# sandeep06011991/OCC-GNN

Measured on AMD Instinct MI355X. Metric: sampled_edges_per_sec, higher is better.
Workload: dtype u32; 1 GPU; products-like synthetic (N=2449029, mean degree 50.5, pareto degrees, seed 0), GraphSAGE fanout 15/10/5 (layer 0 = seeds' hop), minibatch 1024, 4 parts (v % 4), engine-only (sample+slice); streams=128, round_overlap=True, device_lists=int32 (host exports widen to the reference's int64), engine_device_bytes=16549793524

## Files before the change

occ-gnn_amd/csrc/cslicer_hip.hip:

```cpp
#include <hip/hip_runtime.h>

#include <cstdarg>
#include <cstdio>
#include <cstdlib>
#include <cstring>
#include <algorithm>
#include <deque>
#include <vector>

#include "cslicer_hip.h"

namespace {

constexpr uint32_t UNSET = 0xFFFFFFFFu;

constexpr int TN = 256;
#ifdef CSL_OCC7
#define CSL_LB256 __launch_bounds__(256)
#else
#define CSL_LB256 __launch_bounds__(256, 8)
#endif
constexpr int CSL_MAX_SETS = 4;
constexpr int NW = TN / 64;
#ifndef CSL_TPB
// ... 37 lines not shown
       KN_EMIT, KN_SELFIN, KN_MT, KN_EDGES, KN_DUPSEEDS, KN_SELFIN_DEGREE };
const char* const kKernelNames[CSL_NUM_KERNELS] = {"k_seeds",   "k_degree", "k_scan_need", "k_sample",
                                                   "k_scan_buckets", "k_scatter", "k_bucket", "k_count",
                                                   "k_scan_lists", "k_emit",  "k_selfin",  "k_mt19937_fill",
                                                   "k_graph", "k_dupseeds", "k_selfin_degree"};

struct LArgs {
  const unsigned long long* rowinfo;
  const uint32_t* off32;
  const uint32_t* indices;
  const uint8_t* wl;
  uint32_t N, P;
  const uint32_t* ring;
  unsigned long long ring_mask, gen_lo, gen_hi;
  unsigned long long* rngpos;
  unsigned long long* rngbase;
  unsigned long long* acc;
  const uint32_t* fr_in;
  uint32_t* fr_out;
  size_t fr_in_stride, fr_out_stride;
  uint32_t fr_out_cap;
  unsigned long long* ninfo;
  uint32_t* hasedge;
  uint32_t* selfpos;
  uint32_t* firstpos;
  size_t fcap;
  uint32_t* cand;
  uint8_t* cflag;
  uint32_t* crank;
  uint2* queue;
  size_t ccap;
  uint32_t* nbk;
  uint32_t* bcnt;
  uint32_t* bcur;
  uint32_t nbmax;
  uint32_t* tcnt;
  uint32_t tmax, nk;
  uint32_t* fsize;
  csl_sample_meta* meta;
  int* arena;
  size_t arena_stride;
  size_t list_base[CSL_NUM_LISTS];
  uint32_t layer, fanout, W;
  unsigned long long wmagic;
  uint32_t S;
  uint32_t tpb;
  uint32_t* boff;
  uint32_t* ticket;
  uint32_t pmagic;
  uint32_t pmask;
  uint32_t last;
  uint32_t* dupflag;
  uint32_t* seedrep;
  uint32_t* dupfirst;
  uint32_t* dupout;
  size_t fcap0;
  unsigned long long* rngend;
  uint32_t* candk;
  uint32_t graph;
  uint8_t* ecnt;
  uint32_t* srcpos;
  uint32_t* tcur;
};

constexpr uint32_t SELF_BIT = 0x80000000u;
constexpr int kNoReplaceMaxFanout = 64;

__device__ __forceinline__ uint32_t mod_parts(const LArgs& a, uint32_t v) {
  uint32_t r = v - __umulhi(v, a.pmagic) * a.P;
  if (r >= a.P) r -= a.P;
  if (r >= a.P) r -= a.P;
  return r;
}
__device__ __forceinline__ uint32_t owner(const LArgs& a, uint32_t v) {
  return a.wl ? (uint32_t)a.wl[v] : mod_parts(a, v);
}
__device__ __forceinline__ unsigned long long row_lookup(const LArgs& a, uint32_t v) {
  if (a.off32) {
    const uint32_t lo = a.off32[v], hi = a.off32[v + 1];
    return ((unsigned long long)lo << 24) | (unsigned long long)(hi - lo);
  }
  return a.rowinfo[v];
}
__device__ __forceinline__ uint32_t lane_id() { return threadIdx.x & 63; }
__device__ __forceinline__ uint32_t div_w(const LArgs& a, uint32_t c) {
  return (uint32_t)(((unsigned long long)c * a.wmagic) >> 40);
}
__device__ __forceinline__ bool xcd_block_at(const LArgs& a, uint32_t id, uint32_t grid, uint32_t& x, uint32_t& s) {
  const uint32_t groups = (a.S + 7u) >> 3;
  const uint32_t per_stream = grid / (8u * groups);
  const uint32_t j = id >> 3;
  const uint32_t sl = j / per_stream;
  x = j - sl * per_stream;
  s = sl * 8u + (id & 7u);
  return s < a.S;
}
__device__ __forceinline__ bool xcd_block(const LArgs& a, uint32_t& x, uint32_t& s) {
  return xcd_block_at(a, blockIdx.x, gridDim.x, x, s);
}
__device__ __forceinline__ void st_sc1(uint32_t* p, uint32_t v) {
  __hip_atomic_store(p, v, __ATOMIC_RELAXED, __HIP_MEMORY_SCOPE_AGENT);
}
__device__ __forceinline__ uint32_t ld_sc1(const uint32_t* p) {
  return __hip_atomic_load(p, __ATOMIC_RELAXED, __HIP_MEMORY_SCOPE_AGENT);
}
__device__ __forceinline__ bool last_block_of_stream(uint32_t* ticket, uint32_t expected) {
  __shared__ uint32_t s_last;
  asm volatile("s_waitcnt vmcnt(0)" ::: "memory");
  __syncthreads();
  if (threadIdx.x == 0) {
    const uint32_t t = __hip_atomic_fetch_add(ticket, 1u, __ATOMIC_RELAXED, __HIP_MEMORY_SCOPE_AGENT);
    s_last = t == expected - 1u;
    if (t == expected - 1u) {
      st_sc1(ticket, 0u);
      __builtin_amdgcn_fence(__ATOMIC_ACQUIRE, "agent");
      asm volatile("s_waitcnt vmcnt(0)" ::: "memory");
    }
  }
  __syncthreads();
  return s_last != 0u;
}
__device__ __forceinline__ unsigned long long lt_mask() {
  return (1ull << lane_id()) - 1ull;
}
__device__ __forceinline__ uint32_t bucket_of(uint32_t v, uint32_t nb) {
  return __umulhi(v * 0x9E3779B1u, nb);
}
__device__ __forceinline__ uint32_t pass_of(uint32_t v, uint32_t npass) {
  uint32_t x = v * 0x27D4EB2Fu;
  x ^= x >> 13;
  return __umulhi(x * 0x165667B1u, npass);
}
__device__ __forceinline__ uint32_t slot_of(uint32_t v) {
  uint32_t x = v * 0x85EBCA6Bu;
  x ^= x >> 15;
  x *= 0xC2B2AE35u;
  return x >> (32 - HLOG);
}

__device__ __forceinline__ uint32_t wave_excl_scan(uint32_t x, uint32_t& total) {
  uint32_t incl = x;
  for (int o = 1; o < 64; o <<= 1) {
    uint32_t y = __shfl_up(incl, o);
    if ((int)lane_id() >= o) incl += y;
  }
  total = __shfl(incl, 63);
  return incl - x;
}

__device__ __forceinline__ uint32_t wave_incl_scan_dpp(uint32_t x) {
  int v = (int)x;
  v += __builtin_amdgcn_update_dpp(0, v, 0x111, 0xf, 0xf, false);
  v += __builtin_amdgcn_update_dpp(0, v, 0x112, 0xf, 0xf, false);
  v += __builtin_amdgcn_update_dpp(0, v, 0x114, 0xf, 0xf, false);
  v += __builtin_amdgcn_update_dpp(0, v, 0x118, 0xf, 0xf, false);
  v += __builtin_amdgcn_update_dpp(0, v, 0x142, 0xa, 0xf, false);
  v += __builtin_amdgcn_update_dpp(0, v, 0x143, 0xc, 0xf, false);
  return (uint32_t)v;
}
__device__ __forceinline__ uint32_t spread4(uint32_t x) { return ((x & 0xFu) * 0x00204081u) & 0x01010101u; }

constexpr int SCAN_CH = 12;

template <int PHASE>
__device__ __forceinline__ void scan_body(const LArgs& a, const int s) {
  const uint32_t F = ld_sc1(&a.fsize[s * (CSL_MAX_LAYERS + 1) + a.layer]);
// ... 336 lines not shown
      run += h;
      if (bx == 0) boff[b] = grun;
      grun += gcnt[b];
    }
    if (bx == 0 && n == TN - 1) boff[nb] = grun;
  }
  __syncthreads();
  for (uint32_t k0 = n; k0 < cnt; k0 += TN * CU) {
    uint32_t v[CU];
#pragma unroll
    for (int u = 0; u < CU; u++) v[u] = k0 + u * TN < cnt ? cand[k0 + u * TN] : UNSET;
#pragma unroll
    for (int u = 0; u < CU; u++) {
      if (v[u] == UNSET) continue;
      const uint32_t c = (uint32_t)base + k0 + u * TN;
      const uint32_t i = div_w(a, c);
      const uint32_t b = bucket_of(v[u], nb);
      const uint32_t p = s_loff[b] + atomicAdd(&s_hist[b], 1u);
      s_stage[p] = make_uint2(v[u], c == i * W ? (SELF_BIT | i) : c);
    }
  }
  __syncthreads();
  uint2* q = a.queue + (size_t)s * a.ccap;
  const uint32_t staged = s_loff[nb - 1] + s_hist[nb - 1];
  for (uint32_t k = n; k < staged; k += TN) {
    const uint2 e = s_stage[k];
    const uint32_t b = bucket_of(e.x, nb);
    q[s_gbase[b] + (k - s_loff[b])] = e;
  }
}

__device__ __forceinline__ uint32_t ht_find(const uint32_t* h_key, uint32_t val) {
  uint32_t h = slot_of(val);
  for (uint32_t probes = 0; probes < (uint32_t)HCAP; probes++) {
    const uint32_t k = h_key[h];
    if (k == val) return h;
    if (k == UNSET) return UNSET;
    h = (h + 1) & (HCAP - 1);
  }
  return UNSET;
}

#ifndef CSL_BT
#define CSL_BT 512
#endif
#ifndef CSL_RC
#define CSL_RC 4
#endif
constexpr int BT = CSL_BT;
constexpr int RC = CSL_RC;

__device__ __forceinline__ uint32_t ht_insert(uint32_t* h_key, uint32_t val) {
  uint32_t h = slot_of(val);
  for (uint32_t probes = 0; probes < (uint32_t)HCAP; probes++) {
    uint32_t kk = h_key[h];
    if (kk == UNSET) kk = atomicCAS(&h_key[h], UNSET, val);
    if (kk == UNSET || kk == val) return h;
    h = (h + 1) & (HCAP - 1);
  }
  return UNSET;
}

#ifndef CSL_BPB
#define CSL_BPB 4
#endif
constexpr int BPB = CSL_BPB;

__device__ unsigned long long g_wave_dup[3];

template <bool HAS_WL, bool PROBE = false>
__global__ __launch_bounds__(BT) void k_bucket(LArgs a) {
  uint32_t bx, s;
  if (!xcd_block(a, bx, s)) return;
  const uint32_t nbk = a.nbk[s];
  uint32_t b = bx * BPB;
  if (b >= nbk) return;
  __shared__ __attribute__((aligned(16))) uint32_t h_key[HCAP];
  __shared__ __attribute__((aligned(16))) uint32_t h_epos[HCAP];
  __shared__ __attribute__((aligned(16))) uint32_t h_self[HCAP];
  const uint32_t n = threadIdx.x;
  const uint32_t* off = a.boff + (size_t)s * (a.nbmax + 1);
  const uint2* qs = a.queue + (size_t)s * a.ccap;
  const uint32_t W = a.W;
  uint32_t q0 = off[b], q1 = off[b + 1];
  uint2 e[RC];
#pragma unroll
  for (int r = 0; r < RC; r++) e[r] = n + r * BT < q1 - q0 ? qs[q0 + n + r * BT] : make_uint2(UNSET, 0u);
  auto record = [&](const uint2 ee, const uint32_t h) {
    if (ee.y & SELF_BIT) {
      atomicMin(&h_self[h], ee.y & ~SELF_BIT);
      if (a.graph) atomicMin(&h_epos[h], (ee.y & ~SELF_BIT) * W);
    } else {
      atomicMin(&h_epos[h], ee.y);
    }
  };
  auto insert = [&](const uint2 ee) -> uint32_t {
    const uint32_t h = ht_insert(h_key, ee.x);
    if (h == UNSET) {
      atomicOr(&a.meta[s].error, (uint32_t)CSL_ERR_BUCKET_FULL);
    } else {
      record(ee, h);
    }
    return h;
  };
  uint8_t* cflag = a.cflag + (size_t)s * a.ccap;
  auto part_of = [&](const uint32_t v) -> uint32_t { return HAS_WL ? (uint32_t)a.wl[v] : mod_parts(a, v); };
  auto judge = [&](const uint2 ee, const uint32_t epos, const uint32_t self, const uint32_t g) {
    if (ee.y & SELF_BIT) {
      const uint32_t i = ee.y & ~SELF_BIT;
      const uint32_t c = i * W;
      if (self != i) {
        if (a.graph) atomicOr(&a.meta[s].error, (uint32_t)CSL_ERR_DUP_SEED);
        else a.dupflag[s] = 1u;
      }
      if (a.graph) {
        const uint32_t fe = epos == c;
        if (!fe) cflag[c] = 0;
        a.firstpos[s * a.fcap + i] = epos;
      } else {
        const uint32_t newf = epos > c && self == i;
        if (!newf) cflag[c] = 0;
        if (a.layer == 0) a.seedrep[s * a.fcap0 + i] = self;
        if (epos != UNSET) a.firstpos[s * a.fcap + i] = epos;
      }
    } else {
      const uint32_t c = ee.y;
      const uint32_t fe = epos == c;
      if (!fe) {
        cflag[c] = 0;
      } else if (!a.graph && self != UNSET) {
        const uint32_t newf = (unsigned long long)self * W > c;
        cflag[c] = (uint8_t)(newf | 2u | (g << 2) | 32u);
      }
      if (a.graph && !fe) a.srcpos[(size_t)s * a.ccap + c] = epos;
    }
  };
  auto evaluate = [&](const uint2 ee, const uint32_t h) { judge(ee, h_epos[h], h_self[h], part_of(ee.x)); };
  for (int j = 0; j < BPB; j++, b++) {
    if (b >= nbk) break;
    const uint2* q = qs + q0;
    const uint32_t cnt = q1 - q0;
    if (PROBE) {
      unsigned n_e = 0, n_row = 0, n_all = 0;
      const uint32_t lane = lane_id();
#pragma unroll
      for (int r = 0; r < RC; r++) {
        bool later_row = false, later_all = false;
        for (uint32_t sl = 0; sl < 64; sl++) {
#pragma unroll
          for (int r2 = 0; r2 < RC; r2++) {
            const uint32_t other = __shfl(e[r2].x, sl);
            if (other == e[r].x && (r2 < r || (r2 == r && sl < lane))) {
              later_all = true;
              if (r2 == r) later_row = true;
            }
          }
        }
        if (e[r].x != UNSET) {
          n_e++;
          n_row += later_row;
          n_all += later_all;
        }
      }
      atomicAdd(&g_wave_dup[0], (unsigned long long)n_e);
      atomicAdd(&g_wave_dup[1], (unsigned long long)n_row);
      atomicAdd(&g_wave_dup[2], (unsigned long long)n_all);
    }
    uint2 en[RC];
    const bool more = j + 1 < BPB && b + 1 < nbk;
    const uint32_t q1n = off[more ? b + 2 : b + 1];
#pragma unroll
    for (int r = 0; r < RC; r++) {
      const uint32_t k = n + r * BT;
      const bool ok = more && k < q1n - q1;
      en[r] = qs[ok ? q1 + k : 0u];
      if (!ok) en[r] = make_uint2(UNSET, 0u);
    }
    auto clear_table = [&]() {
      const uint4 u4 = make_uint4(UNSET, UNSET, UNSET, UNSET);
      for (uint32_t i = n; i < (uint32_t)HCAP / 4; i += BT) {
        reinterpret_cast<uint4*>(h_key)[i] = u4;
        reinterpret_cast<uint4*>(h_epos)[i] = u4;
        reinterpret_cast<uint4*>(h_self)[i] = u4;
      }
    };
    if (cnt > (uint32_t)HCAP) {
      const uint32_t npass = (cnt + (uint32_t)HCAP / 2 - 1) / ((uint32_t)HCAP / 2);
      for (uint32_t pass = 0; pass < npass; pass++) {
        clear_table();
        __syncthreads();
        for (uint32_t k = n; k < cnt; k += BT) {
          const uint2 ee = q[k];
          if (pass_of(ee.x, npass) == pass) insert(ee);
        }
        __syncthreads();
        for (uint32_t k = n; k < cnt; k += BT) {
          const uint2 ee = q[k];
          if (pass_of(ee.x, npass) != pass) continue;
          const uint32_t h = ht_find(h_key, ee.x);
          if (h != UNSET) evaluate(ee, h);
        }
        __syncthreads();
      }
    } else {
    clear_table();
    __syncthreads();
    uint32_t hs[RC];
#pragma unroll
    for (int r = 0; r < RC; r++) hs[r] = e[r].x != UNSET ? insert(e[r]) : UNSET;
    for (uint32_t k = n + RC * BT; k < cnt; k += BT) insert(q[k]);
    __syncthreads();
    {
      uint32_t og[RC], ep[RC], sf[RC];
#pragma unroll
      for (int r = 0; r < RC; r++) {
// ... 13 lines not shown
    }
    if (!more) break;
    __syncthreads();
#pragma unroll
    for (int r = 0; r < RC; r++) e[r] = en[r];
    q0 = q1;
    q1 = q1n;
  }
}

__device__ __forceinline__ void count_tile(const LArgs& a, const uint32_t s, const uint32_t tile, const uint32_t F);

constexpr int CNT_T = 1024;
__global__ __launch_bounds__(CNT_T) void k_count(LArgs a) {
  uint32_t bx, s;
  if (!xcd_block(a, bx, s)) return;
  const uint32_t F = a.fsize[s * (CSL_MAX_LAYERS + 1) + a.layer];
  const uint32_t tile = bx * (CNT_T / 64) + (threadIdx.x >> 6);
  if (tile * TN < F) count_tile(a, s, tile, F);
  const uint32_t per_stream = gridDim.x / (8u * ((a.S + 7u) >> 3));
  uint32_t nb_act = ((F + TN - 1) / TN + CNT_T / 64 - 1) / (CNT_T / 64);
  if (nb_act < 1) nb_act = 1;
  if (nb_act > per_stream) nb_act = per_stream;
  if (bx >= nb_act) return;
  if (last_block_of_stream(a.ticket + 2 * s + 1, nb_act)) scan_body<1>(a, (int)s);
}

__device__ __forceinline__ void count_tile(const LArgs& a, const uint32_t s, const uint32_t tile, const uint32_t F) {
  const uint32_t W = a.W, P = a.P;
  const uint32_t nodes_here = (F - tile * TN) < (uint32_t)TN ? (F - tile * TN) : (uint32_t)TN;
  const uint32_t nbytes = nodes_here * W;
  const uint32_t* fw = reinterpret_cast<const uint32_t*>(a.cflag + (size_t)s * a.ccap + (size_t)tile * TN * W);
  uint32_t c_new = 0;
  unsigned long long acc_lo = 0, acc_hi = 0;
  for (uint32_t o = lane_id() * 4; o < nbytes; o += 256) {
    uint32_t w = fw[o >> 2];
    if (o + 4 > nbytes) w &= 0xFFFFFFFFu >> (8 * (o + 4 - nbytes));
    c_new += __popc(w & 0x01010101u);
#pragma unroll
    for (int b = 0; b < 4; b++) {
      const uint32_t fl = (w >> (8 * b)) & 0xFFu;
      const unsigned long long one = (unsigned long long)((fl >> 1) & 1u) << (16u * ((fl >> 2) & 3u));
      if (P > 4 && (fl & 16u)) acc_hi += one; else acc_lo += one;
    }
  }
  uint32_t cnt[1 + CSL_MAX_PARTS];
  if (nbytes < 65536u) {
    for (int o = 32; o > 0; o >>= 1) {
      c_new += __shfl_down(c_new, o);
      acc_lo += __shfl_down(acc_lo, o);
      if (P > 4) acc_hi += __shfl_down(acc_hi, o);
    }
    cnt[0] = c_new;
#pragma unroll
    for (int g = 0; g < 4; g++) {
      cnt[1 + g] = (uint32_t)(acc_lo >> (16 * g)) & 0xFFFFu;
      cnt[5 + g] = (uint32_t)(acc_hi >> (16 * g)) & 0xFFFFu;
    }
  } else {
    cnt[0] = c_new;
#pragma unroll
    for (int g = 0; g < 4; g++) {
      cnt[1 + g] = (uint32_t)(acc_lo >> (16 * g)) & 0xFFFFu;
      cnt[5 + g] = (uint32_t)(acc_hi >> (16 * g)) & 0xFFFFu;
    }
#pragma unroll
    for (int k = 0; k < 1 + CSL_MAX_PARTS; k++) {
      uint32_t x = cnt[k];
      for (int o = 32; o > 0; o >>= 1) x += __shfl_down(x, o);
      cnt[k] = x;
    }
  }
  if (lane_id() == 0) {
#pragma unroll
    for (int k = 0; k < 1 + CSL_MAX_PARTS; k++)
      if (k < 1 + (int)P) st_sc1(&a.tcnt[((size_t)s * a.nk + (K_NEWF + k)) * a.tmax + tile], cnt[k]);
  }
}

#ifndef CSL_EP
#define CSL_EP 8
#endif
constexpr int EP = CSL_EP;

__global__ CSL_LB256 void k_emit(LArgs a) {
  uint32_t tile, s;
  if (!xcd_block(a, tile, s)) return;
  const uint32_t F = a.fsize[s * (CSL_MAX_LAYERS + 1) + a.layer];
  if (tile * TN >= F) return;
  const uint32_t n = threadIdx.x;
  const uint32_t w = __builtin_amdgcn_readfirstlane(n >> 6);
  const uint32_t lane = lane_id();
  const uint32_t W = a.W, P = a.P;
  const csl_layer_meta& m = a.meta[s].layer[a.layer];
  int* ar = a.arena + (size_t)s * a.arena_stride;
  const uint32_t* tc = a.tcnt + (size_t)s * a.nk * a.tmax;
#define TB(kind) tc[(size_t)(kind)*a.tmax + tile]
  static_assert(NW == 4, "four wave counts per word");
  __shared__ uint32_t s_wc[2][1 + CSL_MAX_PARTS];
  __shared__ uint32_t s_run[2][1 + CSL_MAX_PARTS];
  __shared__ uint32_t s_wn[5 * 2 * NW];
  const uint32_t below = (1u << (8u * w)) - 1u;
#define WBYTE(word) (reinterpret_cast<uint8_t*>(&(word))[w])
#define BYTESUM(x) __builtin_amdgcn_sad_u8((x), 0u, 0u)
  __shared__ uint32_t s_tb[5 * CSL_MAX_PARTS];
  __shared__ uint32_t s_mo[6][CSL_MAX_PARTS];
  if (n < 1 + P) s_run[0][n] = n == 0 ? TB(K_NEWF) : TB(K_IN(P, n - 1));
  if (n >= 64 && n < 64 + 5 * P) s_tb[n - 64] = TB(K_OUT(P, 0) + (n - 64));
  if (n >= 128 && n < 128 + 6 * CSL_MAX_PARTS) {
    const uint32_t k6 = (n - 128) / CSL_MAX_PARTS, g = (n - 128) % CSL_MAX_PARTS;
    const int list = k6 == 0 ? CSL_IN_NODES : k6 == 1 ? CSL_OUT_NODES : k6 == 2 ? CSL_OWNED_OUT_NODES
                   : k6 == 3 ? CSL_SELF_IDS_OUT : k6 == 4 ? CSL_TO_IDS : CSL_FROM_IDS;
    s_mo[k6][g] = g < P ? m.off[list][g] : 0u;
  }
  const uint32_t i = tile * TN + n;
  const bool act = i < F;
  uint32_t v = 0, hb = 0;
  if (act) {
    v = a.fr_in[s * a.fr_in_stride + i];
    hb = a.hasedge[s * a.fcap + i];
  }
  const uint32_t nodes_here = (F - tile * TN) < (uint32_t)TN ? (F - tile * TN) : (uint32_t)TN;
  const uint32_t ncand = nodes_here * W;
  const uint32_t iters = (ncand + TN - 1) / TN;
  const size_t cbase = (size_t)s * a.ccap + (size_t)tile * TN * W;
  const uint32_t nf_cap = m.next_frontier;
  const unsigned long long lt = lt_mask();
  uint32_t* fr_out = a.fr_out + s * a.fr_out_stride;
  unsigned long long* ninfo = a.ninfo + s * a.fcap;
  int* in_list = ar + a.list_base[CSL_IN_NODES];
  const uint8_t* __restrict__ cflag = a.cflag;
  const uint32_t* __restrict__ cand = a.cand;
  for (uint32_t c0 = 0; c0 < iters; c0 += EP) {
    uint32_t pf[EP], pv[EP];
#pragma unroll
    for (int j = 0; j < EP; j++) {
      const uint32_t k = (c0 + j) * TN + n;
      pf[j] = k < ncand ? cflag[cbase + k] : 0u;
      pv[j] = k < ncand ? cand[cbase + k] : 0u;
    }
#pragma unroll
    for (int j = 0; j < EP; j++) {
      if (c0 + j >= iters) break;
      const uint32_t b = j & 1;
      const uint32_t fl = pf[j], val = pv[j];
      const uint32_t newf = fl & 1u, fe = (fl >> 1) & 1u, g = (fl >> 2) & 7u;
      const unsigned long long m0 = __ballot(newf);
      const uint32_t r0 = __popcll(m0 & lt);
      uint32_t rE = 0;
      if (lane == 0) WBYTE(s_wc[b][0]) = (uint8_t)__popcll(m0);
#pragma unroll
      for (uint32_t gg = 0; gg < CSL_MAX_PARTS; gg++) {
        if (gg < P) {
          const unsigned long long mg = __ballot(fe && g == gg);
          if (g == gg) rE = __popcll(mg & lt);
          if (lane == 0) WBYTE(s_wc[b][1 + gg]) = (uint8_t)__popcll(mg);
        }
      }
      __syncthreads();
      if (n < 1 + P) s_run[b ^ 1][n] = s_run[b][n] + BYTESUM(s_wc[b][n]);
      if (newf) {
        const uint32_t p = s_run[b][0] + r0 + BYTESUM(s_wc[b][0] & below);
        if (p < nf_cap) {
          fr_out[p] = val;
          if (!a.last) ninfo[p] = row_lookup(a, val);
        }
      }
#ifndef CSL_ABLATE_EMIT_IN
      if (fe && ((a.pmask >> g) & 1u)) {
        const uint32_t p = s_run[b][1 + g] + rE + BYTESUM(s_wc[b][1 + g] & below);
        in_list[s_mo[0][g] + p] = (int)val;
        if (a.tcur) a.tcur[(size_t)s * a.ccap + s_mo[0][g] + p] = 0;
        if (a.graph || (fl & 32u)) a.crank[cbase + (c0 + j) * TN + n] = p;
      }
#endif
    }
  }
  static_assert(EP % 2 == 0, "buffer parity");
  const uint32_t to = act ? owner(a, v) : 0u;
  const uint32_t ob = act ? 1u << to : 0u;
  const uint32_t oth = hb & ~ob;
  const bool hi = P > 4;
  const uint32_t one_to = act ? 1u << (8u * (to & 3u)) : 0u;
  const bool to_hi = to >= 4;
  uint32_t wd[5][2];
  wd[0][0] = spread4(hb);
  wd[4][0] = spread4(oth);
  wd[1][0] = (!to_hi && (hb & ob)) ? one_to : 0u;
  wd[2][0] = !to_hi ? one_to : 0u;
  wd[3][0] = (!to_hi && oth) ? one_to : 0u;
  wd[0][1] = wd[1][1] = wd[2][1] = wd[3][1] = wd[4][1] = 0;
  if (hi) {
    wd[0][1] = spread4(hb >> 4);
    wd[4][1] = spread4(oth >> 4);
    wd[1][1] = (to_hi && (hb & ob)) ? one_to : 0u;
    wd[2][1] = to_hi ? one_to : 0u;
    wd[3][1] = (to_hi && oth) ? one_to : 0u;
  }
#pragma unroll
  for (int k = 0; k < 5; k++) {
#pragma unroll
    for (int h = 0; h < 2; h++) {
      if (h == 0 || hi) {
        const uint32_t incl = wave_incl_scan_dpp(wd[k][h]);
        if (lane == 63) s_wn[(k * 2 + h) * NW + w] = incl;
        wd[k][h] = incl - wd[k][h];
      }
    }
  }
  __syncthreads();
  const uint32_t m0 = w > 0 ? 0xFFFFFFFFu : 0u, m1 = w > 1 ? 0xFFFFFFFFu : 0u, m2 = w > 2 ? 0xFFFFFFFFu : 0u;
#pragma unroll
  for (int k = 0; k < 5; k++) {
#pragma unroll
    for (int h = 0; h < 2; h++) {
      if (h == 0 || hi) {
        const uint32_t* c = &s_wn[(k * 2 + h) * NW];
        wd[k][h] += (c[0] & m0) + (c[1] & m1) + (c[2] & m2);
      }
    }
  }
#define RANK(k, g) ((wd[k][(g) >> 2] >> (8u * ((g)&3u))) & 0xFFu)
#ifndef CSL_ABLATE_EMIT_NODES
  if (act) {
    int outrank_to = -1;
#pragma unroll
    for (uint32_t g = 0; g < CSL_MAX_PARTS; g++) {
      if (g < P && ((hb >> g) & 1u)) {
        const uint32_t p = RANK(0, g) + s_tb[0 * P + g];
        if (g == to) outrank_to = p;
        if (!((a.pmask >> g) & 1u)) continue;
        ar[a.list_base[CSL_OUT_NODES] + s_mo[1][g] + p] = (int)v;
        if (g != to && !a.graph) {
          const uint32_t q = RANK(4, g) + s_tb[4 * P + g];
          ar[a.list_base[CSL_FROM_IDS] + s_mo[5][g] + q] = (int)p;
        }
      }
    }
    const uint32_t tsh = 8u * (to & 3u);
#define RANK_TO(k) (((to_hi ? wd[k][1] : wd[k][0]) >> tsh) & 0xFFu)
    const bool mine = (a.pmask >> to) & 1u;
    {
      const uint32_t q = RANK_TO(2) + s_tb[2 * P + to];
      const uint32_t pos = s_mo[3][to] + q;
      if (mine) ar[a.list_base[CSL_SELF_IDS_OUT] + pos] = outrank_to;
      a.selfpos[s * a.fcap + i] = mine ? pos : UNSET;
    }
    if (outrank_to >= 0 && mine) {
      const uint32_t q = RANK_TO(1) + s_tb[1 * P + to];
      ar[a.list_base[CSL_OWNED_OUT_NODES] + s_mo[2][to] + q] = outrank_to;
    }
    if (!a.graph && oth != 0 && mine) {
      const uint32_t q = RANK_TO(3) + s_tb[3 * P + to];
      ar[a.list_base[CSL_TO_IDS] + s_mo[4][to] + q] = outrank_to;
    }
#undef RANK_TO
  }
#else
  if (act) a.selfpos[s * a.fcap + i] = 0;
#endif
#undef RANK
#undef TB
#undef WBYTE
#undef BYTESUM
}

constexpr int DS_T = 256;
__device__ __forceinline__ uint32_t ds_ld(const uint32_t* p) {
  return __hip_atomic_load(p, __ATOMIC_RELAXED, __HIP_MEMORY_SCOPE_AGENT);
}
template <bool IS_MAX>
__device__ __forceinline__ uint32_t ds_block_scan(uint32_t x, uint32_t* s_w, uint32_t& total) {
  const uint32_t lane = lane_id(), w = threadIdx.x >> 6;
  uint32_t incl = x;
  for (int o = 1; o < 64; o <<= 1) {
    const uint32_t y = __shfl_up(incl, o);
    if ((int)lane >= o) incl = IS_MAX ? (incl > y ? incl : y) : incl + y;
  }
  uint32_t excl = __shfl_up(incl, 1);
  if (lane == 0) excl = 0;
  __syncthreads();
  if (lane == 63) s_w[w] = incl;
  __syncthreads();
  uint32_t before = 0, all = 0;
  for (uint32_t k = 0; k < DS_T / 64; k++) {
    const uint32_t t = s_w[k];
    if (k < w) before = IS_MAX ? (before > t ? before : t) : before + t;
    all = IS_MAX ? (all > t ? all : t) : all + t;
  }
  total = all;
  return IS_MAX ? (excl > before ? excl : before) : excl + before;
}

__global__ __launch_bounds__(DS_T) void k_dupseeds(LArgs a) {
  const uint32_t s = blockIdx.x;
  if (!a.dupflag[s]) return;
  const uint32_t F = a.fsize[s * (CSL_MAX_LAYERS + 1)], P = a.P, n = threadIdx.x;
  const uint32_t* fr = a.fr_in + s * a.fr_in_stride;
  const uint32_t* hbv = a.hasedge + s * a.fcap;
  const uint32_t* rep = a.seedrep + s * a.fcap0;
  uint32_t* firstg = a.dupfirst + (size_t)s * a.fcap0 * P;
  uint32_t* outidx = a.dupout + (size_t)s * a.fcap0 * P;
  uint32_t* selfpos = a.selfpos + s * a.fcap;
  int* ar = a.arena + (size_t)s * a.arena_stride;
  csl_layer_meta& m = a.meta[s].layer[0];
  __shared__ uint32_t s_w[DS_T / 64];
  __shared__ uint32_t s_cnt[6][CSL_MAX_PARTS];
  __shared__ uint32_t s_off[5][CSL_MAX_PARTS + 1];
  for (uint32_t k = n; k < F * P; k += DS_T) firstg[k] = UNSET;
  __syncthreads();
  for (uint32_t i = n; i < F; i += DS_T) {
    const uint32_t h = hbv[i], r = rep[i];
    for (uint32_t g = 0; g < P; g++)
      if ((h >> g) & 1u) atomicMin(&firstg[(size_t)r * P + g], i);
  }
  __syncthreads();
  const uint32_t chunks = (F + DS_T - 1) / DS_T;
  for (int pass = 0; pass < 2; pass++) {
    for (uint32_t g = 0; g < P; g++) {
      for (int kind = pass == 0 ? 0 : 1; kind < (pass == 0 ? 6 : 5); kind++) {
        uint32_t run = 0, prev_run = 0;
        for (uint32_t ch = 0; ch < chunks; ch++) {
          const uint32_t i = ch * DS_T + n;
          const bool act = i < F;
          uint32_t v = 0, h = 0, r = 0, to = 0;
          if (act) {
            v = fr[i];
            h = hbv[i];
            r = rep[i];
// ... 855 lines not shown
    a.graph = e->cfg.mode == CSL_MODE_GRAPH ? 1u : 0u;
    a.ecnt = e->ecnt ? e->ecnt + sF * e->P : nullptr;
    a.srcpos = e->srcpos ? e->srcpos + sC : nullptr;
    a.tcur = (e->tcur && (l < L - 1 || (e->cfg.flags & CSL_FLAG_TRANSPOSE_ALL))) ? e->tcur + sC : nullptr;
    a.dupflag = e->dupflag + (size_t)set * S;
    a.fcap0 = e->fcap[0];
    a.seedrep = e->seedrep + (size_t)set * S * e->fcap[0];
    a.dupfirst = e->dupfirst ? e->dupfirst + (size_t)set * S * e->fcap[0] * e->P : nullptr;
    a.dupout = e->dupout ? e->dupout + (size_t)set * S * e->fcap[0] * e->P : nullptr;
    a.rngend = e->rngend + (size_t)set * S;
    a.candk = e->candk ? e->candk + ((size_t)slot * L + l) * S * e->ccap_max : nullptr;
  }
  const dim3 blk(TN);
  const unsigned xg = 8u * (unsigned)((S + 7) / 8);
  auto tiles_of = [&](int l) { return (unsigned)((e->fcap[l] + TN - 1) / TN); };
  auto degree_blocks = [&](int l) { return xg * ((tiles_of(l) + NW - 1) / NW); };
  if (e->nsets > 1 && e->chain_valid) HIPCHECK(hipStreamWaitEvent(st, e->chain_event, 0));
  {
    Timed t(e, KN_DEGREE, st);
    hipLaunchKernelGGL(k_degree, dim3(degree_blocks(0)), blk, 0, st, A[0], nodes_dev, (const BatchDesc*)dd);
  }
  for (int l = 0; l < L; l++) {
    const LArgs& a = A[l];
    const unsigned tiles_in = tiles_of(l);
    const size_t ccap_l = (size_t)tiles_in * TN * a.W;
    const dim3 grid_in(xg * tiles_in);
    const dim3 grid_sample(xg * ((tiles_in + a.tpb - 1) / a.tpb));
    const dim3 grid_scatter(xg * (unsigned)((ccap_l + SCT - 1) / SCT));
    unsigned nb_l = (unsigned)((ccap_l + QMEAN - 1) / QMEAN);
    if (nb_l > e->nbmax) nb_l = e->nbmax;
    const dim3 grid_bucket(xg * ((nb_l + BPB - 1) / BPB));
    const size_t lds_hist = (size_t)e->nbmax * sizeof(uint32_t);
    if (l == L - 1 && e->nsets > 1) {
      HIPCHECK(hipEventRecord(e->chain_event, st));
      e->chain_valid = true;
    }
    {
      Timed t(e, KN_SAMPLE, st);
      static const size_t lds_pad = getenv("CSL_SAMPLE_LDS_PAD") ? (size_t)atol(getenv("CSL_SAMPLE_LDS_PAD")) : 0;
      if (e->cfg.flags & CSL_FLAG_NO_REPLACE)
        hipLaunchKernelGGL(k_sample_norep, grid_sample, blk, lds_hist + lds_pad, st, a);
      else
        hipLaunchKernelGGL(k_sample, grid_sample, blk, lds_hist + lds_pad, st, a);
    }
    if (l == L - 1) {
      const int k = (int)(e->rounds_submitted % csl_engine::NSNAP);
      if (e->snap_pending[k]) {
        int r2 = retire_snapshots(e, e->snap_round[k]);
        if (r2) return r2;
      }
      HIPCHECK(hipMemcpyAsync(e->snap_host + (size_t)k * S, a.rngend, sizeof(unsigned long long) * S,
                              hipMemcpyDeviceToHost, st));
      HIPCHECK(hipEventRecord(e->snap_ev[k], st));
      e->snap_round[k] = e->rounds_submitted;
      e->snap_pending[k] = true;
    }
    {
      Timed t(e, KN_SCATTER, st);
      hipLaunchKernelGGL(k_scatter, grid_scatter, blk, e->scatter_lds, st, a);
    }
    {
      Timed t(e, KN_BUCKET, st);
      static const bool probe = getenv("CSL_WAVE_DUP_PROBE") != nullptr;
      if (probe) hipLaunchKernelGGL((k_bucket<false, true>), grid_bucket, dim3(BT), 0, st, a);
      else if (a.wl) hipLaunchKernelGGL(k_bucket<true>, grid_bucket, dim3(BT), 0, st, a);
      else hipLaunchKernelGGL(k_bucket<false>, grid_bucket, dim3(BT), 0, st, a);
    }
    {
      Timed t(e, KN_COUNT, st);
      hipLaunchKernelGGL(k_count, dim3(xg * ((tiles_in + CNT_T / 64 - 1) / (CNT_T / 64))), dim3(CNT_T), 0, st, a);
    }
    {
      Timed t(e, KN_EMIT, st);
      hipLaunchKernelGGL(k_emit, grid_in, blk, 0, st, a);
    }
    if (a.graph) {
      Timed t(e, KN_EDGES, st);
      hipLaunchKernelGGL(k_graph, grid_in, blk, 0, st, a);
    } else if (l == 0) {
      Timed t(e, KN_DUPSEEDS, st);
      hipLaunchKernelGGL(k_dupseeds, dim3(S), dim3(DS_T), 0, st, a);
    }
    const unsigned n_selfin = xg * ((tiles_in + 3) / 4);
    if (l + 1 < L) {
      Timed t(e, KN_SELFIN_DEGREE, st);
      const unsigned n_degree = degree_blocks(l + 1);
      hipLaunchKernelGGL(k_selfin_degree, dim3(n_degree + n_selfin), blk, 0, st, a, A[l + 1], n_degree);
    } else {
      Timed t(e, KN_SELFIN, st);
      hipLaunchKernelGGL(k_selfin, dim3(n_selfin), blk, 0, st, a);
    }
    if (a.tcur) {
      const unsigned sp = (unsigned)(S * e->P);
      const unsigned in_cap = (unsigned)ccap_l;
      const unsigned ttiles = (in_cap + TT - 1) / TT;
      uint32_t* tsum = e->tsum + (size_t)set * S * e->P * e->ttiles_max;
      hipLaunchKernelGGL(k_tsum, dim3(ttiles, sp), blk, 0, st, a, tsum, (uint32_t)e->ttiles_max);
      hipLaunchKernelGGL(k_tptr, dim3(ttiles, sp), blk, 0, st, a, (const uint32_t*)tsum, (uint32_t)e->ttiles_max);
      hipLaunchKernelGGL(k_tfill, dim3((unsigned)((e->list_cap[l][CSL_OUT_NODES] + TN - 1) / TN), sp), blk, 0, st, a);
      hipLaunchKernelGGL(k_tsort, dim3((in_cap + TN - 1) / TN, sp), blk, 0, st, a);
    }
  }
  HIPCHECK(hipGetLastError());
  for (int s = 0; s < n_batches && s < S; s++) e->pos_ub[s] += e->worst_draws;
  e->rounds_submitted++;
  HIPCHECK(hipEventRecord(e->slot_event[slot], st));
  e->slot_pending[slot] = 1;
  e->dirty = true;
  e->meta_valid[slot] = 0;
  return 0;
}

}

extern "C" {

const char* csl_last_error(void) { return g_err; }
int csl_abi_version(void) { return CSL_ABI_VERSION; }
int csl_noreplace_max_fanout(void) { return kNoReplaceMaxFanout; }
const char* csl_kernel_name(int32_t k) { return (k >= 0 && k < CSL_NUM_KERNELS) ? kKernelNames[k] : ""; }

int csl_debug_wave_duplicates(uint64_t* out3) {
  if (!out3) return CSL_E_INVALID;
  unsigned long long v[3];
  if (hipDeviceSynchronize() != hipSuccess || hipMemcpyFromSymbol(v, HIP_SYMBOL(g_wave_dup), sizeof(v)) != hipSuccess)
    return CSL_E_HIP;
  for (int i = 0; i < 3; i++) out3[i] = v[i];
  return CSL_OK;
}

void csl_destroy(csl_engine* e) {
  if (!e) return;
  hipSetDevice(e->cfg.device);
  for (int k = 0; k < CSL_MAX_SETS; k++)
    if (e->streams[k]) hipStreamSynchronize(e->streams[k]);
  if (e->rng_stream) hipStreamSynchronize(e->rng_stream);
  for (auto& te : e->timed) {
    hipEventDestroy(te.a);
    hipEventDestroy(te.b);
  }
  for (auto ev : e->event_pool) hipEventDestroy(ev);
  void* ptrs[] = {e->rowinfo, e->off32, e->indices, e->wl,      e->nodes, e->seedbuf, e->ring,  e->mt_state, e->rngpos,
                  e->rngbase, e->ninfo,   e->hasedge, e->selfpos, e->firstpos, e->cand, e->cflag, e->crank,
                  e->queue,   e->nbk,     e->bcnt,    e->bcur,    e->tcnt,     e->fsize, e->meta, e->desc_dev,
                  e->ecnt,    e->srcpos,  e->tcur, e->tsum, e->acc,     e->dupflag, e->seedrep, e->dupfirst, e->dupout, e->rngend,
                  e->candk,   e->boff,    e->ticket};
  for (void* p : ptrs)
    if (p) hipFree(p);
  for (int l = 0; l <= CSL_MAX_LAYERS; l++)
    if (e->fr[l]) hipFree(e->fr[l]);
  for (int l = 0; l < CSL_MAX_LAYERS; l++)
    if (e->arena[l]) hipFree(e->arena[l]);
  if (e->desc_host) hipHostFree(e->desc_host);
  for (int k = 0; k < 2; k++)
    if (e->fetch_stage2[k]) hipHostFree(e->fetch_stage2[k]);
  if (e->fetch_pack) hipFree(e->fetch_pack);
  free(e->fetch_host);
  if (e->copy_stream) hipStreamDestroy(e->copy_stream);
  if (e->rng_event) hipEventDestroy(e->rng_event);
  if (e->chain_event) hipEventDestroy(e->chain_event);
  for (auto& c : e->rng_chunks) hipEventDestroy(c.ev);
  for (auto ev : e->rng_event_pool) hipEventDestroy(ev);
  for (int k = 0; k < csl_engine::NSNAP; k++)
    if (e->snap_ev[k]) hipEventDestroy(e->snap_ev[k]);
  if (e->snap_host) hipHostFree(e->snap_host);
  for (auto ev : e->slot_event) hipEventDestroy(ev);
  for (auto ev : e->desc_event) hipEventDestroy(ev);
// ... 620 lines not shown
```

occ-gnn_amd/csrc/k_sample_body.inc:

```
  extern __shared__ __attribute__((aligned(16))) uint32_t s_bh[];
  uint32_t bx, s;
  if (!xcd_block(a, bx, s)) return;
  const uint32_t F = a.fsize[s * (CSL_MAX_LAYERS + 1) + a.layer];
  if (bx * a.tpb * TN >= F) return;
  __shared__ uint32_t s_v[TN];
  __shared__ unsigned long long s_ri[TN];
  __shared__ uint32_t s_rng[TN];
  __shared__ uint32_t s_hb[TN];
  __shared__ uint8_t s_to[TN];
  __shared__ uint32_t s_wn[NW];
  __shared__ uint32_t s_cnt[5 * CSL_MAX_PARTS];
  __shared__ uint32_t s_ec[TN * CSL_MAX_PARTS];
  __shared__ uint32_t s_gcnt[CSL_MAX_PARTS + CSL_MAX_PARTS * CSL_MAX_PARTS];
  const uint32_t n = threadIdx.x;
  const uint32_t f = a.fanout, W = a.W;
  const uint32_t P = a.P;
  const uint32_t nb = a.nbk[s];
  for (uint32_t b = n; b < nb; b += TN) s_bh[b] = 0;
  const unsigned long long rbase = a.rngbase[s];
  for (uint32_t sub = 0; sub < a.tpb; sub++) {
    const uint32_t tile = bx * a.tpb + sub;
    if (tile * TN >= F) break;
    const uint32_t i = tile * TN + n;
    uint32_t v = 0, need = 0;
    unsigned long long ri = 0;
    if (i < F) {
      v = a.fr_in[s * a.fr_in_stride + i];
      ri = a.ninfo[s * a.fcap + i];
      need = (uint32_t)(ri & DEG_MASK) >= f;
    }
    const unsigned long long bm = __ballot(need);
    __syncthreads();
    if (lane_id() == 0) s_wn[n >> 6] = __popcll(bm);
    if (n < 5 * CSL_MAX_PARTS) s_cnt[n] = 0;
    s_v[n] = v;
    s_ri[n] = ri;
    s_hb[n] = 0;
    s_to[n] = i < F ? (uint8_t)owner(a, v) : 0;
    if (a.graph) {
      for (uint32_t k = n; k < TN * P; k += TN) s_ec[k] = 0;
      if (n < CSL_MAX_PARTS + CSL_MAX_PARTS * CSL_MAX_PARTS) s_gcnt[n] = 0;
    }
    __syncthreads();
    {
      uint32_t r = __popcll(bm & lt_mask());
      for (uint32_t w = 0; w < (n >> 6); w++) r += s_wn[w];
      const uint32_t tb = a.tcnt[((size_t)s * a.nk + K_NEED) * a.tmax + tile];
      s_rng[n] = need ? (tb + r) * f : UNSET;
    }
    __syncthreads();
    const uint32_t nodes_here = (F - tile * TN) < (uint32_t)TN ? (F - tile * TN) : (uint32_t)TN;
    const uint32_t ncand = nodes_here * W;
    const size_t cbase = (size_t)s * a.ccap + (size_t)tile * TN * W;
    constexpr int SU = CSL_SU;
    const uint32_t dq = TN / W, dr = TN - dq * W;
    uint32_t nn = n / W, slot = n - nn * W;
    for (uint32_t k0 = n; k0 < ncand; k0 += TN * SU) {
      uint32_t nnu[SU], slu[SU], vvu[SU], degu[SU], val[SU], rnd[SU];
      unsigned long long addr[SU], rpos[SU];
      bool live[SU], gat[SU], rq[SU];
#pragma unroll
      for (int u = 0; u < SU; u++) {
        live[u] = k0 + u * TN < ncand;
        nnu[u] = nn;
        slu[u] = slot;
        nn += dq;
        slot += dr;
        if (slot >= W) {
          slot -= W;
          nn++;
        }
        val[u] = UNSET;
        gat[u] = false;
        rq[u] = false;
        addr[u] = 0;
        rpos[u] = 0;
        vvu[u] = 0;
        degu[u] = 1;
        rnd[u] = 0;
        if (live[u]) {
          vvu[u] = s_v[nnu[u]];
          if (slu[u] == 0) {
            val[u] = vvu[u];
          } else {
            const unsigned long long r2 = s_ri[nnu[u]];
            const uint32_t deg = (uint32_t)(r2 & DEG_MASK);
            const uint32_t j = slu[u] - 1;
            degu[u] = deg;
            addr[u] = r2 >> DEG_BITS;
            if (deg < f) {
              gat[u] = j < deg;
              addr[u] += j;
            } else {
              gat[u] = true;
              rq[u] = true;
              rpos[u] = rbase + s_rng[nnu[u]] + j;
            }
          }
        }
      }
#pragma unroll
      for (int u = 0; u < SU; u++) {
        if (rq[u]) {
          if (rpos[u] >= a.gen_lo && rpos[u] < a.gen_hi) {
            rnd[u] = a.ring[rpos[u] & a.ring_mask];
          } else {
            atomicOr(&a.meta[s].error, (uint32_t)CSL_ERR_RNG_WINDOW);
          }
        }
      }
#pragma unroll
      for (int u = 0; u < SU; u++) {
        if constexpr (NOREP) {
          if (gat[u])
            val[u] = a.indices[addr[u] + (rq[u] ? floyd_pick(a, s, rpos[u] - (slu[u] - 1u), slu[u] - 1u, degu[u] - f, rnd[u]) : 0u)];
        } else {
          if (gat[u]) val[u] = a.indices[addr[u] + (rq[u] ? rnd[u] % degu[u] : 0u)];
        }
      }
#pragma unroll
      for (int u = 0; u < SU; u++) {
        if (live[u]) {
          uint32_t fl = 0;
          if (slu[u] == 0) {
            atomicAdd(&s_bh[bucket_of(val[u], nb)], 1u);
            fl = (a.graph ? 3u : 1u) | ((uint32_t)s_to[nnu[u]] << 2);
          } else if (val[u] != UNSET) {
            if (val[u] == vvu[u]) {
              if (a.candk) a.candk[cbase + k0 + u * TN] = val[u];
              val[u] = UNSET;
            } else {
              const uint32_t og = owner(a, val[u]);
              atomicOr(&s_hb[nnu[u]], 1u << og);
              if (a.graph) atomicAdd(&s_ec[nnu[u] * P + og], 1u);
              atomicAdd(&s_bh[bucket_of(val[u], nb)], 1u);
              fl = 3u | (og << 2);
              if (a.graph) a.srcpos[cbase + k0 + u * TN] = tile * TN * W + k0 + u * TN;
            }
          }
          a.cand[cbase + k0 + u * TN] = val[u];
          a.cflag[cbase + k0 + u * TN] = (uint8_t)fl;
          if (a.candk && (val[u] != UNSET || slu[u] == 0 || !gat[u])) a.candk[cbase + k0 + u * TN] = val[u];
        }
      }
    }
    __syncthreads();
    uint32_t hb = 0, to = 0;
    const bool act = i < F;
    if (act) {
      hb = s_hb[n];
      to = s_to[n];
      if (!a.graph) a.firstpos[s * a.fcap + i] = UNSET;
      if (a.graph) hb |= 1u << to;
      a.hasedge[s * a.fcap + i] = hb;
    }
    if (a.graph) {
      for (uint32_t g = 0; g < P; g++) {
        const uint32_t ec = act ? s_ec[n * P + g] : 0u;
        if (act) a.ecnt[(s * a.fcap + i) * P + g] = (uint8_t)ec;
        uint32_t x = ec;
        for (int o = 32; o > 0; o >>= 1) x += __shfl_down(x, o);
        if (lane_id() == 0 && x) atomicAdd(&s_gcnt[g], x);
        const bool hasg = act && ((hb >> g) & 1u) && to != g;
        for (uint32_t p = 0; p < P; p++) {
          const uint32_t c_pair = __popcll(__ballot(hasg && to == p));
          if (lane_id() == 0 && c_pair) atomicAdd(&s_gcnt[CSL_MAX_PARTS + g * CSL_MAX_PARTS + p], c_pair);
        }
      }
    }
    for (uint32_t g = 0; g < P; g++) {
      const bool own = act && to == g;
      const bool has = act && ((hb >> g) & 1u);
      const uint32_t c_out = __popcll(__ballot(has));
      const uint32_t c_owned = __popcll(__ballot(own && has));
      const uint32_t c_self = __popcll(__ballot(own));
      const uint32_t c_to = __popcll(__ballot(own && (hb & ~(1u << g)) != 0));
      const uint32_t c_from = __popcll(__ballot(has && !own));
      if (lane_id() == 0) {
        if (c_out) atomicAdd(&s_cnt[0 * CSL_MAX_PARTS + g], c_out);
        if (c_owned) atomicAdd(&s_cnt[1 * CSL_MAX_PARTS + g], c_owned);
        if (c_self) atomicAdd(&s_cnt[2 * CSL_MAX_PARTS + g], c_self);
        if (c_to) atomicAdd(&s_cnt[3 * CSL_MAX_PARTS + g], c_to);
        if (c_from) atomicAdd(&s_cnt[4 * CSL_MAX_PARTS + g], c_from);
      }
    }
    __syncthreads();
    if (n < 5 * P) {
      const uint32_t kind5 = n / P, g = n - kind5 * P;
      a.tcnt[((size_t)s * a.nk + (K_OUT(P, 0) + kind5 * P + g)) * a.tmax + tile] = s_cnt[kind5 * CSL_MAX_PARTS + g];
    }
    if (a.graph) {
      if (n < P) a.tcnt[((size_t)s * a.nk + K_ECNT(P, n)) * a.tmax + tile] = s_gcnt[n];
      if (n < P * P) {
        const uint32_t g = n / P, p = n - g * P;
        a.tcnt[((size_t)s * a.nk + K_PAIR(P, g, p)) * a.tmax + tile] = s_gcnt[CSL_MAX_PARTS + g * CSL_MAX_PARTS + p];
      }
    }
  }
  __syncthreads();
  uint32_t* gcnt = a.bcnt + (size_t)s * (a.nbmax + 1);
  for (uint32_t b = n; b < nb; b += TN) {
    const uint32_t c = s_bh[b];
    if (c) atomicAdd(&gcnt[b], c);
  }
```

Measured before the change: 32.90 billion edges/s.

## Fold self-in index resolution into emit kernel, dropping selfin pass for non-graph layers

For non-graph layers after layer 0, the sample kernel now packs each frontier node's within-tile owner rank into the hasedge word, and the bucket kernel writes the source frontier index into crank plus a sampled flag. The emit kernel then queues owned in-node entries per wave in shared memory and resolves their self_ids_in slot directly, so the separate selfin pass and the firstpos/selfpos writes are no longer needed. The combined k_selfin_degree launch is replaced by plain k_degree. In exchange, emit gains a shared queue, extra gathers, and wave-level barriers, and bit packing in hasedge assumes fewer than 256 parts and small per-tile ranks.

Measured after the change: 33.23 billion edges/s, median of 6. Within noise of the previous version (+1.0%).

```diff
diff --git a/occ-gnn_amd/csrc/cslicer_hip.hip b/occ-gnn_amd/csrc/cslicer_hip.hip
--- a/occ-gnn_amd/csrc/cslicer_hip.hip
+++ b/occ-gnn_amd/csrc/cslicer_hip.hip
@@ -143,6 +143,7 @@
   }
   return a.rowinfo[v];
 }
+__host__ __device__ __forceinline__ bool selfin_folded(const LArgs& a) { return !a.graph && a.layer != 0; }
 __device__ __forceinline__ uint32_t lane_id() { return threadIdx.x & 63; }
 __device__ __forceinline__ uint32_t div_w(const LArgs& a, uint32_t c) {
   return (uint32_t)(((unsigned long long)c * a.wmagic) >> 40);
@@ -645,6 +646,7 @@
   const uint32_t* off = a.boff + (size_t)s * (a.nbmax + 1);
   const uint2* qs = a.queue + (size_t)s * a.ccap;
   const uint32_t W = a.W;
+  const bool fold = selfin_folded(a);
   uint32_t q0 = off[b], q1 = off[b + 1];
   uint2 e[RC];
 #pragma unroll
@@ -684,7 +686,10 @@
         const uint32_t newf = epos > c && self == i;
         if (!newf) cflag[c] = 0;
         if (a.layer == 0) a.seedrep[s * a.fcap0 + i] = self;
-        if (epos != UNSET) a.firstpos[s * a.fcap + i] = epos;
+        if (epos != UNSET) {
+          if (fold) reinterpret_cast<uint8_t*>(a.hasedge + s * a.fcap + i)[3] = 1;
+          else a.firstpos[s * a.fcap + i] = epos;
+        }
       }
     } else {
       const uint32_t c = ee.y;
@@ -694,6 +699,7 @@
       } else if (!a.graph && self != UNSET) {
         const uint32_t newf = (unsigned long long)self * W > c;
         cflag[c] = (uint8_t)(newf | 2u | (g << 2) | 32u);
+        if (fold) a.crank[(size_t)s * a.ccap + c] = self;
       }
       if (a.graph && !fe) a.srcpos[(size_t)s * a.ccap + c] = epos;
     }
@@ -873,6 +879,7 @@
 #define CSL_EP 8
 #endif
 constexpr int EP = CSL_EP;
+constexpr int EQ = 256;
 
 __global__ CSL_LB256 void k_emit(LArgs a) {
   uint32_t tile, s;
@@ -896,6 +903,7 @@
 #define BYTESUM(x) __builtin_amdgcn_sad_u8((x), 0u, 0u)
   __shared__ uint32_t s_tb[5 * CSL_MAX_PARTS];
   __shared__ uint32_t s_mo[6][CSL_MAX_PARTS];
+  __shared__ uint2 s_q[NW][EQ];
   if (n < 1 + P) s_run[0][n] = n == 0 ? TB(K_NEWF) : TB(K_IN(P, n - 1));
   if (n >= 64 && n < 64 + 5 * P) s_tb[n - 64] = TB(K_OUT(P, 0) + (n - 64));
   if (n >= 128 && n < 128 + 6 * CSL_MAX_PARTS) {
@@ -911,6 +919,9 @@
     v = a.fr_in[s * a.fr_in_stride + i];
     hb = a.hasedge[s * a.fcap + i];
   }
+  const bool fold = selfin_folded(a);
+  const bool sampled = (hb >> 24) != 0;
+  hb &= 0xFFu;
   const uint32_t nodes_here = (F - tile * TN) < (uint32_t)TN ? (F - tile * TN) : (uint32_t)TN;
   const uint32_t ncand = nodes_here * W;
   const uint32_t iters = (ncand + TN - 1) / TN;
@@ -922,6 +933,28 @@
   int* in_list = ar + a.list_base[CSL_IN_NODES];
   const uint8_t* __restrict__ cflag = a.cflag;
   const uint32_t* __restrict__ cand = a.cand;
+  uint32_t qn = 0;
+  auto resolve = [&](const uint32_t cnt) {
+    int* selfin = ar + a.list_base[CSL_SELF_IDS_IN];
+    const uint32_t* hasedge_s = a.hasedge + s * a.fcap;
+    const uint32_t* crank_t = a.crank + cbase;
+    __builtin_amdgcn_fence(__ATOMIC_RELEASE, "wavefront");
+    __builtin_amdgcn_wave_barrier();
+    for (uint32_t q0 = 0; q0 < cnt; q0 += 64) {
+      const bool ok = q0 + lane < cnt;
+      const uint2 en = s_q[w][ok ? q0 + lane : 0u];
+      const uint32_t g = en.y >> 20;
+      const uint32_t fi = ok ? crank_t[en.y & 0xFFFFFu] : 0u;
+      uint32_t hw = 0, tb = 0;
+      if (ok) {
+        hw = hasedge_s[fi];
+        tb = tc[(size_t)K_SELF(P, g) * a.tmax + fi / TN];
+      }
+      if (ok) selfin[s_mo[3][g] + tb + ((hw >> 8) & 0xFFu)] = (int)en.x;
+    }
+    __builtin_amdgcn_fence(__ATOMIC_ACQUIRE, "wavefront");
+    __builtin_amdgcn_wave_barrier();
+  };
   for (uint32_t c0 = 0; c0 < iters; c0 += EP) {
     uint32_t pf[EP], pv[EP];
 #pragma unroll
@@ -958,15 +991,33 @@
         }
       }
 #ifndef CSL_ABLATE_EMIT_IN
-      if (fe && ((a.pmask >> g) & 1u)) {
+      const bool in_here = fe && ((a.pmask >> g) & 1u);
+      uint32_t p_in = 0;
+      if (in_here) {
         const uint32_t p = s_run[b][1 + g] + rE + BYTESUM(s_wc[b][1 + g] & below);
+        p_in = p;
         in_list[s_mo[0][g] + p] = (int)val;
         if (a.tcur) a.tcur[(size_t)s * a.ccap + s_mo[0][g] + p] = 0;
-        if (a.graph || (fl & 32u)) a.crank[cbase + (c0 + j) * TN + n] = p;
+        if (!fold && (a.graph || (fl & 32u))) a.crank[cbase + (c0 + j) * TN + n] = p;
+      }
+      if (fold) {
+        const bool park = in_here && (fl & 32u);
+        const unsigned long long m5 = __ballot(park);
+        if (m5) {
+          if (qn + 64u > (uint32_t)EQ) {
+            resolve(qn);
+            qn = 0;
+          }
+          if (park) s_q[w][qn + __popcll(m5 & lt)] = make_uint2(p_in, ((c0 + j) * TN + n) | (g << 20));
+          qn += __popcll(m5);
+        }
       }
 #endif
     }
   }
+#ifndef CSL_ABLATE_EMIT_IN
+  if (fold && qn) resolve(qn);
+#endif
   static_assert(EP % 2 == 0, "buffer parity");
   const uint32_t to = act ? owner(a, v) : 0u;
   const uint32_t ob = act ? 1u << to : 0u;
@@ -1035,7 +1086,8 @@
       const uint32_t q = RANK_TO(2) + s_tb[2 * P + to];
       const uint32_t pos = s_mo[3][to] + q;
       if (mine) ar[a.list_base[CSL_SELF_IDS_OUT] + pos] = outrank_to;
-      a.selfpos[s * a.fcap + i] = mine ? pos : UNSET;
+      if (!fold) a.selfpos[s * a.fcap + i] = mine ? pos : UNSET;
+      else if (mine && !sampled) ar[a.list_base[CSL_SELF_IDS_IN] + pos] = -1;
     }
     if (outrank_to >= 0 && mine) {
       const uint32_t q = RANK_TO(1) + s_tb[1 * P + to];
@@ -2057,7 +2109,13 @@
       hipLaunchKernelGGL(k_dupseeds, dim3(S), dim3(DS_T), 0, st, a);
     }
     const unsigned n_selfin = xg * ((tiles_in + 3) / 4);
-    if (l + 1 < L) {
+    if (selfin_folded(a)) {
+      if (l + 1 < L) {
+        Timed t(e, KN_DEGREE, st);
+        hipLaunchKernelGGL(k_degree, dim3(degree_blocks(l + 1)), blk, 0, st, A[l + 1], (const long long*)nullptr,
+                           (const BatchDesc*)nullptr);
+      }
+    } else if (l + 1 < L) {
       Timed t(e, KN_SELFIN_DEGREE, st);
       const unsigned n_degree = degree_blocks(l + 1);
       hipLaunchKernelGGL(k_selfin_degree, dim3(n_degree + n_selfin), blk, 0, st, a, A[l + 1], n_degree);
diff --git a/occ-gnn_amd/csrc/k_sample_body.inc b/occ-gnn_amd/csrc/k_sample_body.inc
--- a/occ-gnn_amd/csrc/k_sample_body.inc
+++ b/occ-gnn_amd/csrc/k_sample_body.inc
@@ -9,6 +9,7 @@
   __shared__ uint32_t s_hb[TN];
   __shared__ uint8_t s_to[TN];
   __shared__ uint32_t s_wn[NW];
+  __shared__ uint8_t s_wo[NW * CSL_MAX_PARTS];
   __shared__ uint32_t s_cnt[5 * CSL_MAX_PARTS];
   __shared__ uint32_t s_ec[TN * CSL_MAX_PARTS];
   __shared__ uint32_t s_gcnt[CSL_MAX_PARTS + CSL_MAX_PARTS * CSL_MAX_PARTS];
@@ -16,6 +17,7 @@
   const uint32_t f = a.fanout, W = a.W;
   const uint32_t P = a.P;
   const uint32_t nb = a.nbk[s];
+  const bool fold = selfin_folded(a);
   for (uint32_t b = n; b < nb; b += TN) s_bh[b] = 0;
   const unsigned long long rbase = a.rngbase[s];
   for (uint32_t sub = 0; sub < a.tpb; sub++) {
@@ -145,14 +147,13 @@
       }
     }
     __syncthreads();
-    uint32_t hb = 0, to = 0;
+    uint32_t hb = 0, to = 0, rk = 0;
     const bool act = i < F;
     if (act) {
       hb = s_hb[n];
       to = s_to[n];
-      if (!a.graph) a.firstpos[s * a.fcap + i] = UNSET;
+      if (!a.graph && !fold) a.firstpos[s * a.fcap + i] = UNSET;
       if (a.graph) hb |= 1u << to;
-      a.hasedge[s * a.fcap + i] = hb;
     }
     if (a.graph) {
       for (uint32_t g = 0; g < P; g++) {
@@ -173,10 +174,13 @@
       const bool has = act && ((hb >> g) & 1u);
       const uint32_t c_out = __popcll(__ballot(has));
       const uint32_t c_owned = __popcll(__ballot(own && has));
-      const uint32_t c_self = __popcll(__ballot(own));
+      const unsigned long long m_own = __ballot(own);
+      const uint32_t c_self = __popcll(m_own);
+      if (own) rk = __popcll(m_own & lt_mask());
       const uint32_t c_to = __popcll(__ballot(own && (hb & ~(1u << g)) != 0));
       const uint32_t c_from = __popcll(__ballot(has && !own));
       if (lane_id() == 0) {
+        s_wo[(n >> 6) * CSL_MAX_PARTS + g] = (uint8_t)c_self;
         if (c_out) atomicAdd(&s_cnt[0 * CSL_MAX_PARTS + g], c_out);
         if (c_owned) atomicAdd(&s_cnt[1 * CSL_MAX_PARTS + g], c_owned);
         if (c_self) atomicAdd(&s_cnt[2 * CSL_MAX_PARTS + g], c_self);
@@ -185,6 +189,13 @@
       }
     }
     __syncthreads();
+    if (act) {
+      if (fold) {
+        for (uint32_t w = 0; w < (n >> 6); w++) rk += s_wo[w * CSL_MAX_PARTS + to];
+        hb |= rk << 8;
+      }
+      a.hasedge[s * a.fcap + i] = hb;
+    }
     if (n < 5 * P) {
       const uint32_t kind5 = n / P, g = n - kind5 * P;
       a.tcnt[((size_t)s * a.nk + (K_OUT(P, 0) + kind5 * P + g)) * a.tmax + tile] = s_cnt[kind5 * CSL_MAX_PARTS + g];
```
